# ParthaEth/GIF

Hardware: AMD Instinct MI355X
Metric: G+D train-step images/sec at 256x256, batch 32/GPU (higher is better)
Workload: dtype f32

## Files before the change

gif_amd/_lib.py:

```python
import ctypes
import os

import torch

_HERE = os.path.dirname(os.path.abspath(__file__))
LIB_PATH = os.path.join(_HERE, "libgif_hip.so")

c_int, c_i64, c_float, c_void_p = ctypes.c_int, ctypes.c_int64, ctypes.c_float, ctypes.c_void_p


def knob(name, default):
    if os.environ.get("GIF_EXPERIMENTAL", "0") in ("", "0"):
        return default
    return os.environ.get(name, default)
P = c_void_p


class ConvGeom(ctypes.Structure):
    _fields_ = [(n, ctypes.c_int32) for n in ("B", "Hb", "Wb", "Cb", "Hs", "Ws", "Cs", "KH", "KW", "stride", "pad")]


class ConvEpilogue(ctypes.Structure):
    _fields_ = [("in_scale", P), ("out_scale", P), ("bias", P), ("residual", P),
                ("act", ctypes.c_int32), ("slope", c_float), ("gain", c_float),
                ("mask_src", P), ("mask_slope", c_float), ("mask_gain", c_float),
                ("dot_src", P), ("dot", P), ("colsum", P), ("red_ws", P), ("out_f32", ctypes.c_int32)]


class LinearBankSeg(ctypes.Structure):
    _fields_ = [("w", P), ("bias", P), ("s", P), ("gs", P), ("gw", P), ("gbias", P), ("n", ctypes.c_int32), ("reserved", ctypes.c_int32)]


GP, EP = ctypes.POINTER(ConvGeom), ctypes.POINTER(ConvEpilogue)

PROTOTYPES = {
    "gif_last_error": (ctypes.c_char_p, []),
    "gif_abi_version": (c_int, []),
    "gif_f16_overflow_clear": (c_int, [P]),
    "gif_f16_overflow_or_into": (c_int, [P, P]),
    "gif_f16_overflow_watch": (c_int, [c_int]),
    "gif_set_fp32_mfma_mode": (c_int, [c_int]),
    "gif_get_fp32_mfma_mode": (c_int, []),
    "gif_rasterize_workspace_bytes": (c_i64, [c_int, c_int, c_int, c_int]),
    "gif_rasterize_assume_clean_workspace": (c_int, [P, c_int]),
    "gif_rasterize_f32": (c_int, [P, P, P, P, c_int, c_int, c_int, c_int, P, P]),
    "gif_rasterize_colors_f32": (c_int, [P, P, P, P, P, c_int, c_int, c_int, c_int, P, P]),
    "gif_rasterize_f64": (c_int, [P, P, P, P, c_int, c_int, c_int, c_int, P, P]),
    "gif_rasterize_colors_f64": (c_int, [P, P, P, P, P, c_int, c_int, c_int, c_int, P, P]),
    "gif_rasterize_colors_bwd_workspace_bytes": (c_i64, [c_int, c_int, c_int, c_int]),
    "gif_rasterize_colors_bwd_f32": (c_int, [P, P, P, P, P, P, c_int, c_int, c_int, c_int, P, P]),
    "gif_vertex_normals_f32": (c_int, [P, P, P, P, P, c_int, c_int, c_int, P]),
    "gif_vertex_normals_bwd_f32": (c_int, [P, P, P, P, P, P, P, c_int, c_int, c_int, P]),
    "gif_face_gather_bwd_f32": (c_int, [P, P, P, P, c_int, c_int, c_int, P]),
    "gif_antialias_f32": (c_int, [P] * 6 + [c_int] * 5 + [P]),
    "gif_antialias_bwd_workspace_bytes": (c_i64, [c_int, c_int, c_int, c_int]),
    "gif_antialias_bwd_f32": (c_int, [P] * 8 + [c_int] * 5 + [P, P]),
    "gif_antialias_walk_f32": (c_int, [P] * 6 + [c_int] * 6 + [P]),
    "gif_antialias_walk_bwd_f32": (c_int, [P] * 8 + [c_int] * 6 + [P, P]),
    "gif_flame_skin_f32": (c_int, [P] * 7 + [c_int] * 4 + [P]),
# ... 174 lines not shown
```

gif_amd/csrc/conv_igemm.hip:

```cpp
#include <stdlib.h>

#include <atomic>
#include <type_traits>

#include "conv_common.h"
#include "conv_route.h"

namespace {

using gif::f32x16, gif::f32x4, gif::xcd_remap;
using gif::buf_rsrc_t, gif::make_buf_rsrc, gif::buf_load_lds16;

struct GatherParams {
    const void* x;
    const void* wp;
    void* y;
    const float* in_scale;
    const float* out_scale;
    const float* bias;
    const void* residual;
    int B, Hi, Wi, Ci;
    int Ho, Wo, Co;
    int Hp, Wp;
    int os, ooy, oox;
    int is;
    int ntaps, nky, nkx, dy0, ddy, dx0, ddx, ky0, kx0, kstep, KW;
    int RP, CP;
    int act;
    float slope, gain;
    int M;
    int tiles_m, tiles_n;
    int stab_nb, stab_stride;
    const void* zero;
    int m_begin;
    int x3;
    const int* wexp;
    unsigned* gate;
    unsigned gate_gen;
    unsigned* h2_stats;
    const void* mask_src;
    const void* dot_src;
    float mask_slope, mask_gain;
    float* part_cs;
    float* part_dot;
    int part_row0;
    int part_cap;
    int no_split;
    unsigned* sat_flag;
    int out_f32;
    int pair;
    int dense;
    int t2_tx, t2_ty;
};

template <int BM, int BN, int LD, int MT, int NT, typename T = float, int THREADS = 256, bool T2D = false, int LDS_FLOATS = 0, int PFMAX = 4>
__device__ __forceinline__ void conv_epilogue(const GatherParams& p, f32x16 (&acc)[MT][NT], float* smem, int m0, int n0,
                                              int wm0, int wn0, int tid, int li, int lh, int HWp, int t2_b = 0, int t2_oy0 = 0,
                                              int t2_ox0 = 0) {
    const T* const res = static_cast<const T*>(p.residual);
    T* const yout = static_cast<T*>(p.y);
    constexpr int LDC = BN + 4;
    constexpr int ROWTAB = 3;
    constexpr int STAGE_FLOATS = LDS_FLOATS ? LDS_FLOATS : 2 * (BM + BN) * LD;
    constexpr int EPI_CHUNKS = (BM * (LDC + ROWTAB) <= STAGE_FLOATS) ? 1 : (BM / 2 * (LDC + ROWTAB) <= STAGE_FLOATS) ? 2
                               : (BM / 4 * (LDC + ROWTAB) <= STAGE_FLOATS) ? 4 : 8;
    constexpr int CR = BM / EPI_CHUNKS;
    static_assert(CR % 32 == 0 && CR * (LDC + ROWTAB) <= STAGE_FLOATS && CR <= THREADS, "epilogue chunk must fit the staging LDS");
    float* Cs = smem;
    unsigned long long* const roff = reinterpret_cast<unsigned long long*>(Cs + CR * LDC);
    int* const rsmp = reinterpret_cast<int*>(roff + CR);
    constexpr unsigned long long NO_ROW = ~0ull;
    constexpr int C4_ROW = BN / 4;
    constexpr int EROWS = THREADS / C4_ROW;
    constexpr int E_IT = CR / EROWS;
    static_assert(CR % EROWS == 0, "epilogue row mapping");
    const int e_row0 = tid / C4_ROW, e_c = (tid % C4_ROW) * 4;
    const int n = n0 + e_c;
    float4 bias4 = make_float4(0.f, 0.f, 0.f, 0.f);
    if (p.bias && n < p.Co) bias4 = *reinterpret_cast<const float4*>(p.bias + n);
    const T* const msk = static_cast<const T*>(p.mask_src);
    const T* const dsrc = static_cast<const T*>(p.dot_src);
    const bool fused = msk || dsrc || p.part_cs || p.part_dot;
    float4 cs = make_float4(0.f, 0.f, 0.f, 0.f), ds = make_float4(0.f, 0.f, 0.f, 0.f);
    int osb = 0;
    f32x4 osc0 = {1.f, 1.f, 1.f, 1.f}, osc1 = osc0;
    constexpr bool OSC = sizeof(T) == 4;
    if (OSC && p.out_scale && n < p.Co) {
        osb = T2D ? t2_b : (m0 < p.M ? m0 : p.M - 1) / HWp;
        osc0 = *reinterpret_cast<const f32x4*>(p.out_scale + (size_t)osb * p.Co + n);
        osc1 = *reinterpret_cast<const f32x4*>(p.out_scale + (size_t)(osb + 1 < p.B ? osb + 1 : osb) * p.Co + n);
    }
#pragma unroll
    for (int c = 0; c < EPI_CHUNKS; ++c) {
        __syncthreads();
        if (tid < CR) {
            int b, oy, ox;
            bool okr;
            if constexpr (T2D) {
                const int r2 = c * CR + tid;
                b = t2_b; oy = t2_oy0 + (r2 >> 4); ox = t2_ox0 + (r2 & 15);
                okr = oy < p.Hp && ox < p.Wp;
            } else {
                const int m = m0 + c * CR + tid;
                okr = m < p.M;
                const int mm = okr ? m : 0;
                b = mm / HWp;
                const int rr = mm - b * HWp;
                oy = rr / p.Wp; ox = rr - oy * p.Wp;
            }
            roff[tid] = okr ? (unsigned long long)((((size_t)b * p.Ho + (oy * p.os + p.ooy)) * p.Wo + (ox * p.os + p.oox)) * p.Co) : NO_ROW;
            rsmp[tid] = b;
        }
#pragma unroll
        for (int i = 0; i < MT; ++i) {
// ... 38 lines not shown
                            }
                        }
                    }
#pragma unroll
                    for (int k = 0; k < PF; ++k) {
                        if (!ok[k]) continue;
                        float4 v = vv[k];
                        if constexpr (sizeof(T) != 4) v = *reinterpret_cast<const float4*>(Cs + (e_row0 + (it0 + k) * EROWS) * LDC + e_c);
                        if (FUSED && dsrc) {
                            ds.x += v.x * xa[k].x; ds.y += v.y * xa[k].y; ds.z += v.z * xa[k].z; ds.w += v.w * xa[k].w;
                        }
                        if (p.out_scale) {
                            f32x4 d = bs[k] == osb ? os0 : os1;
                            if (!OSC || __builtin_expect(bs[k] > osb + 1, 0)) d = *reinterpret_cast<const f32x4*>(p.out_scale + (size_t)bs[k] * p.Co + n);
                            const float dx = d[0], dy = d[1], dz = d[2], dw = d[3];
                            v.x *= dx; v.y *= dy; v.z *= dz; v.w *= dw;
                        }
                        if (res) {
                            float4 rv = gif::load4(res + off[k]);
                            v.x += rv.x; v.y += rv.y; v.z += rv.z; v.w += rv.w;
                        }
                        v.x += bias4.x; v.y += bias4.y; v.z += bias4.z; v.w += bias4.w;
                        if (p.act) {
                            v.x = (v.x > 0.f ? v.x : v.x * p.slope) * p.gain; v.y = (v.y > 0.f ? v.y : v.y * p.slope) * p.gain;
                            v.z = (v.z > 0.f ? v.z : v.z * p.slope) * p.gain; v.w = (v.w > 0.f ? v.w : v.w * p.slope) * p.gain;
                        }
                        if (FUSED) {
                            if (msk) {
                                const float4 xs = two_src ? xb[k] : xa[k];
                                v.x *= p.mask_gain * (xs.x > 0.f ? 1.f : p.mask_slope); v.y *= p.mask_gain * (xs.y > 0.f ? 1.f : p.mask_slope);
                                v.z *= p.mask_gain * (xs.z > 0.f ? 1.f : p.mask_slope); v.w *= p.mask_gain * (xs.w > 0.f ? 1.f : p.mask_slope);
                            }
                            cs.x += v.x; cs.y += v.y; cs.z += v.z; cs.w += v.w;
                        }
                        {
                            if (sizeof(T) == 2 && p.out_f32) gif::store4(static_cast<float*>(p.y) + off[k], v);
                            else gif::store4_flag(yout + off[k], v, p.sat_flag);
                        }
                    }
                }
            };
            if (fused) rows(std::true_type{});
            else rows(std::false_type{});
        }
    }
    if (p.part_cs || p.part_dot) {
        __syncthreads();
        float4* red = reinterpret_cast<float4*>(smem);
        red[tid] = cs;
        red[THREADS + tid] = ds;
        __syncthreads();
        if (tid < C4_ROW && n < p.Co) {
            float4 a = red[tid], b = red[THREADS + tid];
#pragma unroll 4
            for (int k = 1; k < EROWS; ++k) {
                const float4 a2 = red[k * C4_ROW + tid], b2 = red[THREADS + k * C4_ROW + tid];
                a.x += a2.x; a.y += a2.y; a.z += a2.z; a.w += a2.w;
                b.x += b2.x; b.y += b2.y; b.z += b2.z; b.w += b2.w;
            }
            const int prow_i = p.part_row0 + (m0 - p.m_begin) / BM;
            const size_t prow = (size_t)prow_i * p.Co + n;
            if (prow_i < p.part_cap) {
                if (p.part_cs) *reinterpret_cast<float4*>(p.part_cs + prow) = a;
                if (p.part_dot) *reinterpret_cast<float4*>(p.part_dot + prow) = b;
            }
        }
// ... 1245 lines not shown
    if (wp_fallback) {
        const gif::H2Gate gt = gif::h2_next_gate(s);
        if (gt.err) return gt.err;
        p.gate = gt.word; p.gate_gen = gt.gen;
        p.h2_stats = gif::h2_stats_words();
    }
    return 0;
}
inline void h2_to_fallback(GatherParams& p, const void* wp3) {
    p.x3 = 1;
    p.wp = wp3;
    p.wexp = nullptr;
}

template <typename T>
int check_channels(const gif_conv_geom* g, const char* who) {
    if (sizeof(T) == 2)
        GIF_REQUIRE(g->Cb % 8 == 0 && g->Cs % 8 == 0, "%s: f16 channel counts must be multiples of 8 (Cb=%d Cs=%d)", who, g->Cb, g->Cs);
    return 0;
}

template <typename T>
route::ConvShape conv_shape(const gif_conv_geom* g, const gif_conv_epilogue* e, int x3, bool dense) {
    return route::ConvShape{g->B, g->Hb, g->Wb, g->Cb, g->Hs, g->Ws, g->Cs, g->KH, g->KW, g->stride, g->pad,
                            sizeof(T) == 2, x3, dense, e && e->in_scale, e && e->dot};
}

template <typename T>
int base_params(GatherParams& p, const void* x, const void* wp, void* y, const gif_conv_epilogue* e, int x3, int RP, const void* wp_fallback,
                hipStream_t s) {
    p.x = x; p.wp = wp; p.y = y; p.x3 = x3;
    gif::fill_epilogue(p, e);
    p.in_scale = e ? e->in_scale : nullptr;
    p.sat_flag = nullptr;
    p.out_f32 = e ? e->out_f32 : 0;
    if (sizeof(T) == 2) p.sat_flag = gif::f16_sat_flag();
    return x3 == 2 ? h2_operands(p, RP, wp, wp_fallback, s) : 0;
}

template <typename T>
int conv_run(const GatherParams& base, const route::ConvPhases& phs, const void* wp_fallback, const gif::FusedSums& sums, double flops, int d0, int d3,
             int B, long hw, hipStream_t s, const char* who, const char* twin_note) {
    const bool halo_on = halo_switch().load(std::memory_order_relaxed) != 0;
    const route::ConvRoute r = route::conv_route(phs.ph, phs.nph, sizeof(T) == 2, conv_knobs(), halo_on);
    const bool guarded = base.x3 == 2 && base.gate && wp_fallback;
    route::ConvPhases twin = phs;
    route::ConvRoute r2{};
    if (guarded) {
        for (route::ConvPhase& q : twin.ph) q.x3 = 1;
        r2 = route::conv_route(twin.ph, twin.nph, false, conv_knobs(), halo_on);
        if (!r.error && !r2.error && sums.active() && (r2.part_rows != r.part_rows || r2.tile_rows != r.tile_rows)) {
            gif::set_error("%s: the guarded bf16x3 twin tiles the op differently from the f16x2 launch (%d x %d vs %d x %d rows)%s", who,
                           r2.part_rows, r2.tile_rows, r.part_rows, r.tile_rows, twin_note);
            return GIF_ENOSUP;
        }
    }
    const route::ConvPhase& q0 = phs.ph[0];
    gif::ProfScope prof(r.family, flops, s, d0, q0.Co, q0.Ci, d3);
    GatherParams ph[4];
    for (int i = 0; i < phs.nph; ++i) {
        ph[i] = base;
        fill_phase(ph[i], phs.ph[i]);
    }
    if (r.error) return route_error(r);
    for (int i = 0; i < r.nlaunch; ++i)
        if (int rc = conv_dispatch(r.launch[i], ph, s, who)) return rc;
// ... 157 lines not shown
```

gif_amd/csrc/conv_winograd.hip:

```cpp
#include <stdlib.h>
#include <string.h>

#include "conv_common.h"
#include "wino_route.h"

namespace route = gif_wino;

namespace {

using gif::f32x16, gif::f32x4, gif::xcd_remap;

using route::WBM, route::WBN, route::WBK, route::WNSTAGE;
using route::WPAD;

__global__ void __launch_bounds__(256) wino_input_transform(const float* __restrict__ x, const float* __restrict__ scale,
                                                            float* __restrict__ V, int B, int H, int W, int C, int CP,
                                                            long ntiles_pad) {
    const int C4 = CP >> 2, TH = H >> 1, TW = W >> 1;
    const long ntiles = (long)B * TH * TW;
    const long total = ntiles * C4;
    const size_t plane = (size_t)ntiles_pad * CP;
    for (unsigned idx = blockIdx.x * blockDim.x + threadIdx.x; idx < (unsigned)total; idx += gridDim.x * blockDim.x) {
        const unsigned tile = idx / (unsigned)C4;
        const int c4 = (int)(idx - tile * (unsigned)C4);
// ... 1086 lines not shown
    return true;
}
template <int BM, int BN>
bool x3_try(const route::WinoLaunch& l, hipStream_t s, const WinoParams& p) {
    if (l.kernel != route::GEMM_X3 || l.BM != BM || l.BN != BN) return false;
    static gif::LdsAttr attr;
    gif::launch_lds(wino_gemm_x3<BM, BN>, attr, dim3(l.grid), dim3(l.threads), l.lds, s, p);
    return true;
}
template <int BM, int BN, int NST>
bool h2_try(const route::WinoLaunch& l, hipStream_t s, const WinoParams& p) {
    if (l.kernel != route::GEMM_H2 || l.BM != BM || l.BN != BN || l.NST != NST) return false;
    static gif::LdsAttr attr;
    gif::launch_lds(wino_gemm_h2<BM, BN, NST>, attr, dim3(l.grid), dim3(l.threads), l.lds, s, p);
    return true;
}

int wino_launch_one(const route::WinoLaunch& l, hipStream_t s, const WinoParams& p, const char* who) {
    const bool launched = mfma_try<4>(l, s, p) || mfma_try<2>(l, s, p) ||
                          h2_try<128, 128, 3>(l, s, p) || h2_try<128, 128, 5>(l, s, p) || h2_try<128, 128, 4>(l, s, p) ||
                          x3_try<256, 64>(l, s, p) || x3_try<128, 128>(l, s, p);
    GIF_REQUIRE(launched, "%s: the route names a kernel that is not built (gemm %d wn %d tile %dx%d stages %d)", who, l.kernel, l.WN, l.BM, l.BN,
                l.NST);
    return 0;
}

int conv3x3_winograd_impl(int mode, const float* x, const void* U, const void* U2, float* y, float* V, int B, int H, int W, int C, int Co,
                          const gif_conv_epilogue* e, gif_stream_t stream) {
    const bool split = mode != route::MODE_NATIVE, h2 = mode == route::MODE_F16X2;
    const char* const who = split ? "winograd_x3" : "winograd";
    const char* const entry = split ? "conv3x3_winograd_f32x3" : "conv3x3_winograd";
    GIF_REQUIRE(x && (U || U2) && y && V && B >= 0 && H > 0 && W > 0 && H % 2 == 0 && W % 2 == 0, "%s: bad dims (H, W must be even)", who);
    GIF_REQUIRE(C > 0 && Co > 0 && C % 4 == 0 && Co % 4 == 0, "%s: channels must be multiples of 4", who);
    if (B == 0) return 0;
    const route::WinoRoute r = route::wino_route(B, H, W, C, Co, mode, h2 && U, wino_knobs());
    GIF_REQUIRE(r.error == route::WINO_OK, "%s: tensor too large for 32-bit offsets", who);
    hipStream_t s = gif::as_stream(stream);
    double flops = 2.0 * B * H * W * 9.0 * C * Co;
    {
        gif::ProfScope prof_t(r.xform.family, 4.0 * ((double)B * H * W * C + 16.0 * r.ntiles_pad * r.CP), s, (int)((long)B * H * W), C, 0, 1);
        if (int rc = gif::winograd_input_transform(x, e ? e->in_scale : nullptr, V, B, H, W, C, s)) return rc;
    }
    gif::ProfScope prof(r.family, flops, s, (int)((long)B * H * W), Co, C, split ? 2091 : 1091);
    WinoParams p{};
    p.V = V; p.U = static_cast<const float*>(U); p.y = y;
    gif::fill_epilogue(p, e);
    p.B = B; p.H = H; p.W = W; p.Co = Co; p.RP = r.RP; p.CP = r.CP;
    p.ntiles = (int)r.ntiles; p.ntiles_pad = (int)r.ntiles_pad; p.TH = H / 2; p.TW = W / 2;
    p.tiles_m = r.primary.tiles_m; p.tiles_n = r.primary.tiles_n;
    gif::FusedSums sums;
    if (int rc = sums_begin(sums, p, e, B, H, W, Co, r.sum_tile, entry)) return rc;
    if (h2) {
        WinoParams q = p;
        q.uexp = static_cast<const int*>(U2);
        q.U = reinterpret_cast<const float*>(static_cast<const char*>(U2) + gif::h2_header_bytes(r.RP));
        if (r.has_twin) {
            const gif::H2Gate gt = gif::h2_next_gate(s);
            if (gt.err) return gt.err;
            q.gate = gt.word; q.gate_gen = gt.gen;
        }
        if (int rc = wino_launch_one(r.primary, s, q, entry)) return rc;
        if (!q.gate) {
            if (int rc = sums_finish(sums, p, B, H, W, Co, r.sum_tile, s)) return rc;
            return gif::check_launch("conv3x3_winograd_f32h2");
        }
        p.gate = q.gate; p.gate_gen = q.gate_gen; p.h2_stats = gif::h2_stats_words();
// ... 79 lines not shown
```

gif_amd/csrc/elementwise.hip:

```cpp
#include "common.h"

namespace {

__device__ __forceinline__ float wave_sum(float v) {
#pragma unroll
    for (int off = 32; off > 0; off >>= 1) v += __shfl_xor(v, off, 64);
    return v;
}

__device__ __forceinline__ float4 f4add(float4 a, float4 b) { return make_float4(a.x + b.x, a.y + b.y, a.z + b.z, a.w + b.w); }
__device__ __forceinline__ float4 f4fma(float s, float4 a, float4 c) {
    return make_float4(fmaf(s, a.x, c.x), fmaf(s, a.y, c.y), fmaf(s, a.z, c.z), fmaf(s, a.w, c.w));
}
__device__ __forceinline__ float lrelu(float v, float slope, float gain) { return (v > 0.f ? v : v * slope) * gain; }

template <typename T>
struct UpfirdnParams {
    const T* x;
    const float* k;
    T* y;
    const float* bias;
    const T* residual;
    int B, Hi, Wi, C, Ho, Wo, up, down, padx0, pady0, KH, KW, flip, act;
    float slope, gain;
// ... 583 lines not shown
    const int f = R / S, o0 = f / 2 - 1;
    long total = (long)B * R * R * C4;
    for (long idx = (long)blockIdx.x * blockDim.x + threadIdx.x; idx < total; idx += (long)gridDim.x * blockDim.x) {
        int c4 = (int)(idx % C4);
        long pix = idx / C4;
        int ix = (int)(pix % R);
        long t = pix / R;
        int iy = (int)(t % R), b = (int)(t / R);
        float4 r = make_float4(0.f, 0.f, 0.f, 0.f);
        if (f == 1) {
            r = reinterpret_cast<const float4*>(gy)[idx];
        } else {
            int ry = iy % f - o0, rx = ix % f - o0;
            if ((ry == 0 || ry == 1) && (rx == 0 || rx == 1)) {
                float4 g = reinterpret_cast<const float4*>(gy)[(((size_t)b * S + iy / f) * S + ix / f) * C4 + c4];
                r = make_float4(0.25f * g.x, 0.25f * g.y, 0.25f * g.z, 0.25f * g.w);
            }
        }
        reinterpret_cast<float4*>(gx)[idx] = r;
    }
}

const gif_ew::FirKnobs& fir_knobs() {
    static const gif_ew::FirKnobs once = gif_ew::parse_fir_knobs(gif::knob("GIF_FIR_BLOCK"));
    return once;
}

template <typename T>
int upfirdn2d_impl(const T* x, const float* k, T* y, int B, int Hi, int Wi, int C, int Ho, int Wo, int up, int down, int padx0,
                   int pady0, int KH, int KW, int flip, const gif_conv_epilogue* e, gif_stream_t stream) {
    GIF_REQUIRE(x && k && y, "upfirdn2d: null pointer");
    GIF_REQUIRE(B >= 0 && Hi > 0 && Wi > 0 && Ho > 0 && Wo > 0 && C > 0 && C % 4 == 0, "upfirdn2d: bad dims (C=%d)", C);
    GIF_REQUIRE(up >= 1 && down >= 1 && KH >= 1 && KW >= 1 && KH * KW <= 16, "upfirdn2d: bad up/down/kernel");
    if (B == 0) return 0;
    UpfirdnParams<T> p{};
    p.x = x; p.k = k; p.y = y;
    p.bias = e ? e->bias : nullptr;
    p.residual = e ? static_cast<const T*>(e->residual) : nullptr;
    p.act = e ? e->act : 0;
    p.slope = e ? e->slope : 0.f;
    p.gain = e ? e->gain : 1.f;
    p.B = B; p.Hi = Hi; p.Wi = Wi; p.C = C; p.Ho = Ho; p.Wo = Wo; p.up = up; p.down = down;
    p.padx0 = padx0; p.pady0 = pady0; p.KH = KH; p.KW = KW; p.flip = flip;
    p.sat_flag = sizeof(T) == 2 ? gif::f16_sat_flag() : nullptr;
    float* colsum_out = nullptr;
    if (e && (e->mask_src || e->colsum || e->dot || e->dot_src)) {
        GIF_REQUIRE(!e->dot && !e->dot_src, "upfirdn2d: the dot fusion is a convolution epilogue only");
        GIF_REQUIRE(up == 1 && down == 1 && KH == 4 && KW == 4, "upfirdn2d: mask / colsum fusions need the 4x4 blur form (up = down = 1)");
        GIF_REQUIRE(!e->colsum || (e->red_ws && (C & (C - 1)) == 0 && C <= 1024), "upfirdn2d: colsum needs red_ws and a power-of-two C <= 1024");
        p.mask_src = static_cast<const T*>(e->mask_src);
        p.mask_slope = e->mask_slope; p.mask_gain = e->mask_gain;
        colsum_out = e->colsum;
        p.part_cs = colsum_out ? e->red_ws : nullptr;
    }
    const gif_ew::FirRoute r = gif_ew::fir_route({B, C, Ho, Wo, up, down, padx0, pady0, KH, KW}, colsum_out != nullptr, fir_knobs());
    const dim3 grid(r.grid_x, r.grid_y);
    hipStream_t s = gif::as_stream(stream);
    const char* what = "upfirdn2d";
    switch (r.kernel) {
    case gif_ew::FIR_BLUR_ROWS:
        blur4x4_rows_kernel<T, 16, 4><<<grid, r.threads, 0, s>>>(p);
        what = "upfirdn2d(blur rows)";
        break;
    case gif_ew::FIR_BLUR_TILED:
        blur4x4_tiled_kernel<T, 2, 4><<<grid, r.threads, 0, s>>>(p);
        what = "upfirdn2d(blur)";
// ... 398 lines not shown
```

gif_amd/functional.py:

```python
import weakref

import torch
from torch.autograd import Function

from . import ops
from .ops import ConvSpec


class ActPort:
    __slots__ = ("alias", "slope", "gain", "want_bias", "parts", "y_ref")

    def __init__(self, slope, gain, want_bias):
        self.alias, self.slope, self.gain, self.want_bias = None, float(slope), float(gain), bool(want_bias)
        self.parts = []
        self.y_ref = None

    def cfg(self):
        return (self.slope, self.gain, self.want_bias, self.parts, self.y_ref)


def _observed(t):
    return t.retains_grad or bool(t._backward_hooks)


def _port_live(cfg):
    if cfg is None:
        return False
    y = cfg[4]() if cfg[4] is not None else None
    return y is None or not _observed(y)


def _file_part(parts, part):
    if not parts:
        torch.autograd.Variable._execution_engine.queue_callback(parts.clear)
    parts.append(part)


def _take_port(x, identity=False):
    port = getattr(x, "_gif_port", None)
    if (port is None or not ops.FUSE_GRAD or not torch.is_grad_enabled() or port.alias is None or not port.alias.requires_grad
            or (port.slope == 1.0 and port.gain == 1.0) != identity or _observed(x)):
        return None, None
    return port.alias, port.cfg()


_inputs_only = False


class inputs_only_backward:
    def __enter__(self):
        global _inputs_only
        self._prev, _inputs_only = _inputs_only, True

    def __exit__(self, *exc):
        global _inputs_only
        _inputs_only = self._prev


def _param_mask(*tensors):
    P = torch.nn.Parameter
    return tuple(isinstance(t, torch.Tensor) and (isinstance(t, P) or isinstance(getattr(t, "_base", None), P)) for t in tensors)


def _need(ctx, i):
    return ctx.needs_input_grad[i] and not (_inputs_only and ctx.pmask[i])


def _port_on(ctx):
    return ctx.in_port is not None and not torch.is_grad_enabled() and _port_live(ctx.in_port)


def _tag(y, alias, port):
    if port is not None:
        port.alias = alias
        port.y_ref = weakref.ref(y)
        y._gif_port = port
    return y


def _new_port(x_requires_grad, slope, gain, bias):
    if not ops.FUSE_GRAD or not torch.is_grad_enabled():
        return None
    want_bias = bias is not None and bias.requires_grad
    if slope == 1.0 and gain == 1.0 and not want_bias:
        return None
    return ActPort(slope, gain, want_bias)


def _deliver_residual(r_port, gpre, gb):
    want_b, parts = r_port[2:4]
    if want_b:
        _file_part(parts, gb if gb is not None else ops.colsum(gpre))
    return gpre


def _mask_into_port(cfg, gx, x):
    slope, gain, want_b, parts = cfg[:4]
    gxm, gb = BiasActBwdFn.apply(gx, x, want_b, slope, gain)
    if want_b:
        _file_part(parts, gb)
    return gxm


def _producer_gpre(gy, g_port, y, want_b, slope, gain, parts):
    gpre = gb = None
    if gy is not None:
        gpre, gb = BiasActBwdFn.apply(gy, y, want_b, slope, gain)
        if not want_b:
            gb = None
    if g_port is not None:
        gpre = g_port if gpre is None else gpre + g_port
        if want_b and parts:
            for part in parts:
                gb = part if gb is None else gb + part
    if parts is not None:
        parts.clear()
    return gpre, gb


class Conv2dFn(Function):

    @staticmethod
    def forward(ctx, x, w, spec, transposed, out_hw, wscale, residual=None):
        ctx.pmask = _param_mask(x, w)
        x = ops.nhwc(x)
        ctx.spec, ctx.transposed, ctx.wscale = spec, transposed, wscale
        ctx.save_for_backward(x, w)
        ctx.v = None
        epi = {} if residual is None else {"residual": ops.nhwc(residual)}
        if not transposed:
            y, v = ops.conv_fwd(x, w, spec, wscale, keep_v=True, **epi)
            ctx.v = v if ctx.needs_input_grad[1] else None
            return y
        return ops.conv_bwd_data(x, w, spec, tuple(out_hw), wscale, **epi)

    @staticmethod
    def backward(ctx, gy):
        x, w = ctx.saved_tensors
# ... 36 lines not shown
    def forward(ctx, x, w, bias, spec, wscale, slope, gain, passthrough=False, in_port=None, parts=None, x_port=None):
        ctx.set_materialize_grads(False)
        ctx.pmask = _param_mask(x, w, bias)
        x = ops.nhwc(x)
        y, v = ops.conv_fwd(x, w, spec, wscale, keep_v=True, bias=bias, act=True, slope=slope, gain=gain)
        ctx.v = v if ctx.needs_input_grad[1] else None
        ctx.cfg = (spec, wscale, slope, gain, bias is not None)
        ctx.in_port, ctx.parts = in_port, parts
        ctx.save_for_backward(x, w, y)
        return y, y.detach(), (x.view_as(x) if passthrough else None)

    @staticmethod
    def backward(ctx, gy, g_port=None, g_alias=None):
        x, w, y = ctx.saved_tensors
        spec, ws, slope, gain, has_bias = ctx.cfg
        want_b = has_bias and _need(ctx, 2)
        gx = gw = None
        port = _port_on(ctx)
        gpre, gb = _producer_gpre(gy, g_port, y, want_b, slope, gain, ctx.parts)
        if gpre is not None:
            if ctx.needs_input_grad[0]:
                gx = _conv_dgrad(gpre, w, spec, tuple(x.shape[2:]), ws, g_alias, ctx.in_port if port else None, x)
            if _need(ctx, 1):
                gw = WgradFn.apply(gpre, x, spec, w.shape[0], w.shape[1], ws, ctx.v)
        elif ctx.needs_input_grad[0] and g_alias is not None:
            gx = _mask_into_port(ctx.in_port, g_alias, x) if port else g_alias
        return (None if port else gx), gw, (gb if want_b else None), None, None, None, None, None, None, None, (gx if port else None)


def _conv_dgrad(gpre, w, spec, big_hw, ws, residual, in_port, x):
    if in_port is None:
        return Conv2dFn.apply(gpre, w, spec, True, big_hw, ws, residual)
    slope, gain, want_b, parts = in_port[:4]
    fuse = ops.GradFuse(mask_src=x, mask_slope=slope, mask_gain=gain, want_colsum=want_b)
    gx = ops.conv_bwd_data(gpre, w, spec, big_hw, ws, residual=None if residual is None else ops.nhwc(residual), fuse=fuse)
    if want_b:
        _file_part(parts, fuse.colsum)
    return gx


def conv2d_bias_act(x, w, bias, stride=1, pad=0, wscale=1.0, slope=0.2, gain=2 ** 0.5, passthrough=False):
    x_port, in_port = _take_port(x)
    port = _new_port(True, slope, gain, bias)
    y, alias, x_alias = ConvBiasActFn.apply(x, w, bias, ConvSpec(w.shape[2], w.shape[3], stride, pad), wscale, slope, gain,
                                            bool(passthrough), in_port, None if port is None else port.parts, x_port)
    _tag(y, alias, port)
    return (y, x_alias) if passthrough else y


def conv2d(x, w, stride=1, pad=0, wscale=1.0, residual=None):
    return Conv2dFn.apply(x, w, ConvSpec(w.shape[2], w.shape[3], stride, pad), False, None, wscale, residual)


def conv_transpose2d(x, w, stride, pad, out_hw, wscale=1.0):
    return Conv2dFn.apply(x, w, ConvSpec(w.shape[2], w.shape[3], stride, pad), True, tuple(out_hw), wscale, None)


class LinearNtFn(Function):

    @staticmethod
    def forward(ctx, a, b, scale, n_pad):
        ctx.scale = scale
        ctx.pmask = _param_mask(a, b)
        ctx.save_for_backward(a, b)
        return ops.linear_nt(a, b, None, scale, n_pad=n_pad)

    @staticmethod
    def backward(ctx, g):
        a, b = ctx.saved_tensors
        N, K = b.shape
        ga = LinearNnFn.apply(g, b, ctx.scale, a.shape[1]) if _need(ctx, 0) else None
# ... 400 lines not shown
def minibatch_stddev(x, group, Cy):
    if x.dtype != torch.float32:
        return MbstdFn.apply(x.float(), group, Cy).to(x.dtype)
    return MbstdFn.apply(x, group, Cy)


def _modconv_composite(x, w, s, d, spec, transposed, out_hw, wscale, residual=None, bias=None, act=None):
    z = Conv2dFn.apply(x * s.to(x.dtype)[:, :, None, None], w, spec, transposed, out_hw, wscale, None)
    if d is not None:
        z = z * d.to(z.dtype)[:, :, None, None]
    if act is None:
        return z
    slope, gain = act
    return BiasActFn.apply(z, bias, residual, slope, gain)


def _recorded_backward(inputs, needs, gy, build):
    with torch.enable_grad():
        proxies = [None if t is None else t.view_as(t) for t in inputs]
        y = build(*proxies)
        idx = [i for i, (t, n) in enumerate(zip(inputs, needs)) if n and t is not None and t.requires_grad]
        grads = torch.autograd.grad(y, [proxies[i] for i in idx], gy, create_graph=True, allow_unused=True)
    out = [None] * len(inputs)
    for i, g in zip(idx, grads):
        out[i] = g
    return out


def _modconv_dgrad_fused(g, w, spec, tr, x, s, d, ws, in_port, want_gs):
    slope, gain, want_b, parts = in_port[:4] if in_port is not None else (1.0, 1.0, False, None)
    fuse = None
    if in_port is not None or want_gs:
        fuse = ops.GradFuse(mask_src=x if in_port is not None else None, mask_slope=slope, mask_gain=gain, want_colsum=want_b,
                            dot_src=x if want_gs else None)
    if not tr:
        gx = ops.conv_bwd_data(g, w, spec, tuple(x.shape[2:]), ws, in_scale=d, out_scale=s, fuse=fuse)
    else:
        gx = ops.conv_fwd(g, w, spec, ws, in_scale=d, out_scale=s, fuse=fuse)
    if want_b:
        _file_part(parts, fuse.colsum)
    return gx, (None if fuse is None else fuse.dot)


class ModConvFn(Function):

    @staticmethod
    def forward(ctx, x, w, s, d, spec, transposed, out_hw, wscale, in_port=None, x_port=None, out_f32=False):
        x_in, s_in, d_in = x, s, d
        ctx.pmask = _param_mask(x, w, s, d)
        x = ops.nhwc(x)
        s = s.contiguous()
        d = None if d is None else d.contiguous()
        ctx.v = None
        if not transposed:
            y, v = ops.conv_fwd(x, w, spec, wscale, keep_v=True, in_scale=s, out_scale=d, out_f32=out_f32)
            ctx.v = v if ctx.needs_input_grad[1] else None
        else:
            y = ops.conv_bwd_data(x, w, spec, tuple(out_hw), wscale, in_scale=s, out_scale=d)
        ctx.spec, ctx.transposed, ctx.wscale = spec, transposed, wscale
        ctx.out_hw = tuple(y.shape[2:])
        ctx.in_port = in_port
        none = x.new_empty(())
        ctx.save_for_backward(x_in, w, s_in, d_in if d is not None else none, y if d is not None else none)
        ctx.has_d = d is not None
        return y

    @staticmethod
    def backward(ctx, gy):
        x, w, s, d, y = ctx.saved_tensors
        d = d if ctx.has_d else None
        spec, tr, ws = ctx.spec, ctx.transposed, ctx.wscale
        if torch.is_grad_enabled():
            gx, gw, gs, gd = _recorded_backward(
# ... 114 lines not shown
```

gif_amd/ops.py:

```python
import ctypes
import functools
import os
import weakref
from typing import NamedTuple, Optional

import torch

from . import _lib

CL = torch.channels_last


def _stream():
    return torch.cuda.current_stream().cuda_stream


def _device_guard(fn):
    @functools.wraps(fn)
    def wrapped(*args, **kw):
        dev = None
        for a in args + tuple(kw.values()):
            if isinstance(a, torch.Tensor) and a.is_cuda:
                if dev is None:
                    dev = a.device
# ... 40 lines not shown


def _same_dtype(a, b, what):
    if a.dtype != b.dtype:
        raise _lib.GifHipError(f"{what}: operands of different dtypes ({a.dtype} and {b.dtype})")


def empty_nhwc(B, C, H, W, device, dtype=torch.float32):
    return torch.empty((B, C, H, W), device=device, dtype=dtype, memory_format=CL)


class ConvSpec(NamedTuple):
    KH: int
    KW: int
    stride: int
    pad: int

    def small_hw(self, Hb, Wb):
        return ((Hb + 2 * self.pad - self.KH) // self.stride + 1, (Wb + 2 * self.pad - self.KW) // self.stride + 1)

    def big_hw(self, Hs, Ws):
        return ((Hs - 1) * self.stride + self.KH - 2 * self.pad, (Ws - 1) * self.stride + self.KW - 2 * self.pad)


def _geom(B, Hb, Wb, Cb, Hs, Ws, Cs, spec: ConvSpec):
    return _lib.ConvGeom(B, Hb, Wb, Cb, Hs, Ws, Cs, spec.KH, spec.KW, spec.stride, spec.pad)


FUSE_GRAD = _lib.knob("GIF_FUSE_GRAD", "1") != "0"


class GradFuse:

    def __init__(self, mask_src=None, mask_slope=1.0, mask_gain=1.0, want_colsum=False, dot_src=None):
        self.mask_src, self.mask_slope, self.mask_gain = mask_src, float(mask_slope), float(mask_gain)
        self.want_colsum, self.dot_src = bool(want_colsum), dot_src
        self.colsum = self.dot = self._ws = None


def dot_fusable(H, W, dtype=torch.float32):
    return FUSE_GRAD and dtype in (torch.float32, torch.float16) and (H * W) % 1024 == 0


def _epilogue(in_scale=None, out_scale=None, bias=None, residual=None, act=False, slope=0.2, gain=2 ** 0.5, fuse=None,
              out_bchw=None, dtype=torch.float32, out_f32=False):
    e = _lib.ConvEpilogue(_p(in_scale), _p(out_scale), _p(bias), _p(residual), 1 if act else 0, slope, gain)
    e.out_f32 = 1 if out_f32 else 0
    if fuse is not None:
        B, C, H, W = out_bchw
        for t, what in ((fuse.mask_src, "mask_src"), (fuse.dot_src, "dot_src")):
            if t is not None and (tuple(t.shape) != (B, C, H, W) or t.dtype != dtype or not t.is_contiguous(memory_format=CL)):
                raise _lib.GifHipError(f"GradFuse.{what}: expected an NHWC {dtype} tensor of shape {(B, C, H, W)}, got {tuple(t.shape)} {t.dtype}")
        e.mask_src, e.mask_slope, e.mask_gain = _p(fuse.mask_src), fuse.mask_slope, fuse.mask_gain
        e.dot_src = _p(fuse.dot_src)
        if fuse.mask_src is None and fuse.dot_src is None:
            raise _lib.GifHipError("GradFuse: nothing to fuse (the plain column sum of a gradient is ops.colsum)")
        device = fuse.mask_src.device if fuse.mask_src is not None else fuse.dot_src.device
        if fuse.dot_src is not None:
            fuse.dot = torch.empty((B, C), device=device, dtype=torch.float32)
            e.dot = fuse.dot.data_ptr()
        if fuse.want_colsum:
            fuse.colsum = torch.empty((C,), device=device, dtype=torch.float32)
            e.colsum = fuse.colsum.data_ptr()
        if fuse.dot is not None or fuse.colsum is not None:
            fuse._ws = torch.empty((_lib.load().gif_conv_epilogue_ws_floats(B * H * W, C),), device=device, dtype=torch.float32)
            e.red_ws = fuse._ws.data_ptr()
    return e


WEIGHT_CACHE = _lib.knob("GIF_WEIGHT_CACHE", "1") != "0"
_weight_cache = {}
_WEIGHT_CACHE_MAX = 512


def clear_weight_cache():
    _weight_cache.clear()


def _cached_weight_op(w, tag, build):
    if not WEIGHT_CACHE:
        return build()
    base = w._base if w._base is not None else w
    key = (id(base), tag, w.storage_offset(), tuple(w.shape), tuple(w.stride()))
    state = (base.data_ptr(), base._version)
    hit = _weight_cache.get(key)
    if hit is not None and hit[0]() is base and hit[1] == state:
        return hit[2]
# ... 169 lines not shown

def conv3x3_winograd(x, w, rows_are_out: bool, cout_act: int, wscale=1.0, keep_v=False, **epi):
    global _winograd_calls
    _winograd_calls += 1
    lib = _lib.load()
    x = nhwc(x)
    B, C, H, W = x.shape
    R, Cc, sr, sc, sky, skx = _weight_view(w, rows_are_out, cout_act, C)
    mode = winograd_mode("fwd", cout_act)

    def build():
        RP, CP = _dims(lib.gif_winograd_pack_dims if mode == "native" else lib.gif_winograd_pack_dims_x3, cout_act, C, "winograd_pack_dims")
        U = [torch.empty((lib.gif_winograd_weight_f32h2_bytes(RP, CP),), device=x.device, dtype=torch.uint8)] if mode == "f16x2" else []
        U.append(torch.empty((16, RP, CP), device=x.device, dtype=torch.float32) if mode == "native" else
                 torch.empty((16, 3, RP, CP), device=x.device, dtype=torch.bfloat16))
        _call("winograd_weight", mode, w.data_ptr(), *[u.data_ptr() for u in U], R, Cc, RP, CP, sr, sc, sky, skx, 0 if rows_are_out else 1,
              float(wscale), _stream())
        return tuple(U) if mode == "f16x2" else U[0]

    U = _cached_weight_op(w, ("wino", rows_are_out, cout_act, C, float(wscale), mode), build)
    V = torch.empty((lib.gif_winograd_workspace_floats(B, H, W, C),), device=x.device, dtype=torch.float32)
    out = empty_nhwc(B, cout_act, H, W, x.device)
    e = _epilogue(out_bchw=(B, cout_act, H, W), **epi)
    _call("conv3x3_winograd", mode, x.data_ptr(), *_weight_ptrs(U), out.data_ptr(), V.data_ptr(), B, H, W, C, cout_act, ctypes.byref(e), _stream())
    return (out, V) if keep_v else out


def _epi_check(x, epi):
    r = epi.get("residual")
    if r is not None:
        _same_dtype(x, r, "conv epilogue residual")


def _conv_direct(plan: ConvPlan, op: str, src, w, out_bchw, g, wscale, epi):
    fwd, dt = op == "conv2d_fwd", src.dtype
    if plan.mode == "f16x2":
        wp = pack_weight_h2x3(w, fwd, out_bchw[1], src.shape[1], wscale, tapdense=plan.dense)
    else:
        wp = pack_weight(w, fwd, out_bchw[1], src.shape[1], wscale, dt, x3=plan.mode == "bf16x3", tapdense=plan.dense)
    out = empty_nhwc(*out_bchw, src.device, torch.float32 if epi.get("out_f32") else dt)
    e = _epilogue(out_bchw=out_bchw, dtype=dt, **epi)
    _call(op, plan.mode, src.data_ptr(), *_weight_ptrs(wp), out.data_ptr(), ctypes.byref(g), ctypes.byref(e), _stream(), dense=plan.dense)
    return out


def conv_fwd(big, w, spec: ConvSpec, wscale=1.0, keep_v=False, **epi):
    big = nhwc(big)
    dt = big.dtype
    B, Cb, Hb, Wb = big.shape
    Cs = cpad(w.shape[0], dt)
    Hs, Ws = spec.small_hw(Hb, Wb)
    _epi_check(big, epi)
    if dt != torch.float16:
        epi.pop("out_f32", None)
    plan = conv_plan("fwd", dt, B, spec, (Hb, Wb), (Hs, Ws), Cb, Cs, epi, big.numel() * big.element_size())
    if plan.route == "winograd":
        return conv3x3_winograd(big, w, True, Cs, wscale, keep_v=keep_v, **epi)
    out = _conv_direct(plan, "conv2d_fwd", big, w, (B, Cs, Hs, Ws), _geom(B, Hb, Wb, Cb, Hs, Ws, Cs, spec), wscale, epi)
    return (out, None) if keep_v else out


def conv_bwd_data(small, w, spec: ConvSpec, big_hw, wscale=1.0, **epi):
    small = nhwc(small)
    dt = small.dtype
    B, Cs, Hs, Ws = small.shape
    Cb = cpad(w.shape[1], dt)
    Hb, Wb = big_hw
    _epi_check(small, epi)
    plan = conv_plan("dgrad", dt, B, spec, (Hb, Wb), (Hs, Ws), Cs, Cb, epi, small.numel() * small.element_size())
    if plan.route == "winograd":
        return conv3x3_winograd(small, w, False, Cb, wscale, **epi)
    return _conv_direct(plan, "conv2d_bwd_data", small, w, (B, Cb, Hb, Wb), _geom(B, Hb, Wb, Cb, Hs, Ws, Cs, spec), wscale, epi)


def pad32(c: int) -> int:
    return (c + 31) // 32 * 32


def conv3x3_winograd_wgrad(small, big, O, I, wscale=1.0, small_scale=None, big_scale=None, big_v=None):
    global _winograd_calls
    _winograd_calls += 1
    lib = _lib.load()
    small, big = nhwc(small), nhwc(big)
    B, Cs, H, W = small.shape
    Cb = big.shape[1]
    assert big.shape == (B, Cb, H, W) and O <= Cs and I <= Cb
    RP, CP = _dims(lib.gif_conv2d_wgrad_dims, pad32(Cs), pad32(Cb), "wgrad_dims")
    nsplit = lib.gif_conv3x3_winograd_wgrad_splits(B, H, W, Cs, Cb)
    dev = small.device
    nv = lib.gif_winograd_workspace_floats(B, H, W, Cb)
    if big_v is not None and big_v.numel() != nv:
        raise _lib.GifHipError(f"conv3x3_winograd_wgrad: cached V has {big_v.numel()} floats, expected {nv}")
    V = big_v if big_v is not None else torch.empty((nv,), device=dev, dtype=torch.float32)
    Mg = torch.empty((lib.gif_winograd_workspace_floats(B, H, W, Cs),), device=dev, dtype=torch.float32)
    ws = torch.empty((nsplit, 16, RP, CP), device=dev, dtype=torch.float32)
    _call("conv3x3_winograd_wgrad", winograd_mode("wgrad", Cs), None if big_v is not None else big.data_ptr(), small.data_ptr(), V.data_ptr(),
          Mg.data_ptr(), ws.data_ptr(), _p(small_scale), _p(big_scale), B, H, W, Cs, Cb, nsplit, _stream())
    dw = torch.empty((O, I, 3, 3), device=dev, dtype=torch.float32)
    so, si, sky, skx = dw.stride()
    _lib.check(lib.gif_winograd_unpack_wgrad_f32(ws.data_ptr(), dw.data_ptr(), nsplit, O, I, RP, CP, so, si, sky, skx, float(wscale),
                                                 _stream()), "winograd_unpack_wgrad")
    return dw


# ... 520 lines not shown
```

include/gif_hip.h:

```cpp
#ifndef GIF_HIP_H
#define GIF_HIP_H

#include <stdint.h>

#ifdef __cplusplus
extern "C" {
#endif

#define GIF_EINVAL (-1)
#define GIF_ENOSUP (-2)

typedef void* gif_stream_t;

const char* gif_last_error(void);
int gif_abi_version(void);

int gif_f16_overflow_clear(gif_stream_t stream);
int gif_f16_overflow_or_into(float* found_inf, gif_stream_t stream);
int gif_f16_overflow_watch(int on);

#define GIF_FP32_MFMA_NATIVE 0
#define GIF_FP32_MFMA_BF16X3 1
#define GIF_FP32_MFMA_F16X2 2
int gif_set_fp32_mfma_mode(int mode);
// ... 88 lines not shown
                            const int32_t* texel_map, const int32_t* texel_faces, const float* texel_bc, float* gimg,
                            int B, int C, int H, int W, int V, int T, gif_stream_t stream);

int gif_shade_sh_f32(const float* uv, const float* nrm, const uint8_t* mask, const float* albedo, const float* sh, float* out,
                     int B, int Ba, int H, int W, int T, float nrm_mul, float nrm_add, gif_stream_t stream);
int64_t gif_shade_sh_bwd_workspace_bytes(int B, int H, int W);
int gif_shade_sh_bwd_f32(const float* uv, const float* nrm, const uint8_t* mask, const float* albedo, const float* sh,
                         const float* g_out, float* g_uv, float* g_nrm, float* g_albedo, float* g_sh, int B, int Ba, int H,
                         int W, int T, float nrm_mul, float nrm_add, void* workspace, gif_stream_t stream);

typedef struct {
    int32_t B;
    int32_t Hb, Wb, Cb;
    int32_t Hs, Ws, Cs;
    int32_t KH, KW;
    int32_t stride;
    int32_t pad;
} gif_conv_geom;

typedef struct {
    const float* in_scale;
    const float* out_scale;
    const float* bias;
    const void* residual;
    int32_t act;
    float slope, gain;
    const void* mask_src;
    float mask_slope, mask_gain;
    const void* dot_src;
    float* dot;
    float* colsum;
    float* red_ws;
    int32_t out_f32;
} gif_conv_epilogue;
int64_t gif_conv_epilogue_ws_floats(int64_t out_rows, int cout);

int gif_conv2d_pack_dims(int cout, int cin, int* RP, int* CP);
int gif_pack_weight_f32(const float* w, float* wp, int R, int C, int KH, int KW, int RP, int CP, int64_t sr,
                        int64_t sc, int64_t sky, int64_t skx, float scale, gif_stream_t stream);
int gif_conv2d_fwd_f32(const float* big, const float* wp, float* small, const gif_conv_geom* g,
                       const gif_conv_epilogue* e, gif_stream_t stream);
int gif_conv2d_bwd_data_f32(const float* small, const float* wp, float* big, const gif_conv_geom* g,
                            const gif_conv_epilogue* e, gif_stream_t stream);
int gif_conv2d_fwd_f32x3(const float* big, const void* wp3, float* small, const gif_conv_geom* g, const gif_conv_epilogue* e,
                         gif_stream_t stream);
int gif_conv2d_bwd_data_f32x3(const float* small, const void* wp3, float* big, const gif_conv_geom* g,
                              const gif_conv_epilogue* e, gif_stream_t stream);
int gif_conv2d_fwd_f32h2(const float* big, const void* wp2, const void* wp3, float* small, const gif_conv_geom* g,
                         const gif_conv_epilogue* e, gif_stream_t stream);
int gif_conv2d_bwd_data_f32h2(const float* small, const void* wp2, const void* wp3, float* big, const gif_conv_geom* g,
                              const gif_conv_epilogue* e, gif_stream_t stream);
int gif_conv2d_fwd_f32h2_tapdense(const float* big, const void* wp2, const void* wp3, float* small, const gif_conv_geom* g,
                                  const gif_conv_epilogue* e, gif_stream_t stream);
int gif_conv2d_bwd_data_f32h2_tapdense(const float* small, const void* wp2, const void* wp3, float* big, const gif_conv_geom* g,
                                       const gif_conv_epilogue* e, gif_stream_t stream);
int gif_conv2d_fwd_f32x3_tapdense(const float* big, const void* wp3, float* small, const gif_conv_geom* g,
                                  const gif_conv_epilogue* e, gif_stream_t stream);
int gif_conv2d_bwd_data_f32x3_tapdense(const float* small, const void* wp3, float* big, const gif_conv_geom* g,
                                       const gif_conv_epilogue* e, gif_stream_t stream);
int gif_conv2d_wgrad_dims(int Cs, int Cb, int* RP, int* CP);
int gif_conv2d_wgrad_splits(const gif_conv_geom* g);
int gif_conv2d_wgrad_f32(const float* small, const float* big, float* ws, const float* small_scale,
                         const float* big_scale, const gif_conv_geom* g, int nsplit, gif_stream_t stream);
int gif_conv2d_wgrad_f32x3(const float* small, const float* big, float* ws, const float* small_scale,
                           const float* big_scale, const gif_conv_geom* g, int nsplit, gif_stream_t stream);
int gif_conv2d_wgrad_f32h2(const float* small, const float* big, float* ws, const float* small_scale,
// ... 156 lines not shown
```

Before: 178.7.

## Fuse joining of two masked input gradients into conv dgrad epilogue accumulate

When an activation feeds two consumers, the first consumer's masked input gradient is parked in a pending list and not returned to autograd. The second consumer's conv backward-data kernel then adds it in its epilogue via a new accum pointer. This removes a separate elementwise gradient-sum pass and one full read/write of the tensor. It adds bookkeeping around autograd ordering, falls back to an explicit add in the producer's backward, and is disabled on winograd and upfirdn routes.

```diff
diff --git a/gif_amd/_lib.py b/gif_amd/_lib.py
--- a/gif_amd/_lib.py
+++ b/gif_amd/_lib.py
@@ -24,7 +24,8 @@
     _fields_ = [("in_scale", P), ("out_scale", P), ("bias", P), ("residual", P),
                 ("act", ctypes.c_int32), ("slope", c_float), ("gain", c_float),
                 ("mask_src", P), ("mask_slope", c_float), ("mask_gain", c_float),
-                ("dot_src", P), ("dot", P), ("colsum", P), ("red_ws", P), ("out_f32", ctypes.c_int32)]
+                ("dot_src", P), ("dot", P), ("colsum", P), ("red_ws", P), ("out_f32", ctypes.c_int32),
+                ("accum", P)]
 
 
 class LinearBankSeg(ctypes.Structure):
diff --git a/gif_amd/csrc/conv_igemm.hip b/gif_amd/csrc/conv_igemm.hip
--- a/gif_amd/csrc/conv_igemm.hip
+++ b/gif_amd/csrc/conv_igemm.hip
@@ -43,6 +43,7 @@
     float mask_slope, mask_gain;
     float* part_cs;
     float* part_dot;
+    const void* accum;
     int part_row0;
     int part_cap;
     int no_split;
@@ -80,6 +81,7 @@
     if (p.bias && n < p.Co) bias4 = *reinterpret_cast<const float4*>(p.bias + n);
     const T* const msk = static_cast<const T*>(p.mask_src);
     const T* const dsrc = static_cast<const T*>(p.dot_src);
+    const T* const accum = static_cast<const T*>(p.accum);
     const bool fused = msk || dsrc || p.part_cs || p.part_dot;
     float4 cs = make_float4(0.f, 0.f, 0.f, 0.f), ds = make_float4(0.f, 0.f, 0.f, 0.f);
     int osb = 0;
@@ -184,6 +186,10 @@
                                 v.z *= p.mask_gain * (xs.z > 0.f ? 1.f : p.mask_slope); v.w *= p.mask_gain * (xs.w > 0.f ? 1.f : p.mask_slope);
                             }
                             cs.x += v.x; cs.y += v.y; cs.z += v.z; cs.w += v.w;
+                            if (accum) {
+                                const float4 av = gif::load4(accum + off[k]);
+                                v.x += av.x; v.y += av.y; v.z += av.z; v.w += av.w;
+                            }
                         }
                         {
                             if (sizeof(T) == 2 && p.out_f32) gif::store4(static_cast<float*>(p.y) + off[k], v);
@@ -1495,6 +1501,8 @@
     p.x = x; p.wp = wp; p.y = y; p.x3 = x3;
     gif::fill_epilogue(p, e);
     p.in_scale = e ? e->in_scale : nullptr;
+    p.accum = e ? e->accum : nullptr;
+    GIF_REQUIRE(!p.accum || p.mask_src, "conv2d: accum joins two MASKED gradients: it needs mask_src");
     p.sat_flag = nullptr;
     p.out_f32 = e ? e->out_f32 : 0;
     if (sizeof(T) == 2) p.sat_flag = gif::f16_sat_flag();
diff --git a/gif_amd/csrc/conv_winograd.hip b/gif_amd/csrc/conv_winograd.hip
--- a/gif_amd/csrc/conv_winograd.hip
+++ b/gif_amd/csrc/conv_winograd.hip
@@ -1142,6 +1142,7 @@
     const char* const entry = split ? "conv3x3_winograd_f32x3" : "conv3x3_winograd";
     GIF_REQUIRE(x && (U || U2) && y && V && B >= 0 && H > 0 && W > 0 && H % 2 == 0 && W % 2 == 0, "%s: bad dims (H, W must be even)", who);
     GIF_REQUIRE(C > 0 && Co > 0 && C % 4 == 0 && Co % 4 == 0, "%s: channels must be multiples of 4", who);
+    GIF_REQUIRE(!(e && e->accum), "%s: the post-mask accumulate is an epilogue of the direct convolution kernels only", who);
     if (B == 0) return 0;
     const route::WinoRoute r = route::wino_route(B, H, W, C, Co, mode, h2 && U, wino_knobs());
     GIF_REQUIRE(r.error == route::WINO_OK, "%s: tensor too large for 32-bit offsets", who);
diff --git a/gif_amd/csrc/elementwise.hip b/gif_amd/csrc/elementwise.hip
--- a/gif_amd/csrc/elementwise.hip
+++ b/gif_amd/csrc/elementwise.hip
@@ -639,6 +639,7 @@
     GIF_REQUIRE(x && k && y, "upfirdn2d: null pointer");
     GIF_REQUIRE(B >= 0 && Hi > 0 && Wi > 0 && Ho > 0 && Wo > 0 && C > 0 && C % 4 == 0, "upfirdn2d: bad dims (C=%d)", C);
     GIF_REQUIRE(up >= 1 && down >= 1 && KH >= 1 && KW >= 1 && KH * KW <= 16, "upfirdn2d: bad up/down/kernel");
+    GIF_REQUIRE(!(e && e->accum), "upfirdn2d: the post-mask accumulate is an epilogue of the direct convolution kernels only");
     if (B == 0) return 0;
     UpfirdnParams<T> p{};
     p.x = x; p.k = k; p.y = y;
diff --git a/gif_amd/functional.py b/gif_amd/functional.py
--- a/gif_amd/functional.py
+++ b/gif_amd/functional.py
@@ -7,12 +7,20 @@
 from .ops import ConvSpec
 
 
+class _Parts(list):
+    __slots__ = ("pending", "takers")
+
+    def __init__(self):
+        super().__init__()
+        self.pending, self.takers = [], 0
+
+
 class ActPort:
     __slots__ = ("alias", "slope", "gain", "want_bias", "parts", "y_ref")
 
     def __init__(self, slope, gain, want_bias):
         self.alias, self.slope, self.gain, self.want_bias = None, float(slope), float(gain), bool(want_bias)
-        self.parts = []
+        self.parts = _Parts()
         self.y_ref = None
 
     def cfg(self):
@@ -41,7 +49,26 @@
     if (port is None or not ops.FUSE_GRAD or not torch.is_grad_enabled() or port.alias is None or not port.alias.requires_grad
             or (port.slope == 1.0 and port.gain == 1.0) != identity or _observed(x)):
         return None, None
+    port.parts.takers += 1
     return port.alias, port.cfg()
+
+
+def _join_accum(in_port):
+    pend = in_port[3].pending
+    return pend[0] if pend else None
+
+
+def _join_result(in_port, gx, fuse):
+    parts = in_port[3]
+    pend = parts.pending
+    if fuse.joined:
+        pend.clear()
+        return gx
+    if parts.takers < 2 or pend:
+        return gx
+    torch.autograd.Variable._execution_engine.queue_callback(pend.clear)
+    pend.append(gx)
+    return None
 
 
 _inputs_only = False
@@ -104,6 +131,10 @@
 
 def _producer_gpre(gy, g_port, y, want_b, slope, gain, parts):
     gpre = gb = None
+    pend = getattr(parts, "pending", None)
+    if pend:
+        g_port = pend[0] if g_port is None else g_port + pend[0]
+        pend.clear()
     if gy is not None:
         gpre, gb = BiasActBwdFn.apply(gy, y, want_b, slope, gain)
         if not want_b:
@@ -206,11 +237,11 @@
     if in_port is None:
         return Conv2dFn.apply(gpre, w, spec, True, big_hw, ws, residual)
     slope, gain, want_b, parts = in_port[:4]
-    fuse = ops.GradFuse(mask_src=x, mask_slope=slope, mask_gain=gain, want_colsum=want_b)
+    fuse = ops.GradFuse(mask_src=x, mask_slope=slope, mask_gain=gain, want_colsum=want_b, accum=_join_accum(in_port))
     gx = ops.conv_bwd_data(gpre, w, spec, big_hw, ws, residual=None if residual is None else ops.nhwc(residual), fuse=fuse)
     if want_b:
         _file_part(parts, fuse.colsum)
-    return gx
+    return _join_result(in_port, gx, fuse)
 
 
 def conv2d_bias_act(x, w, bias, stride=1, pad=0, wscale=1.0, slope=0.2, gain=2 ** 0.5, passthrough=False):
@@ -677,13 +708,15 @@
     fuse = None
     if in_port is not None or want_gs:
         fuse = ops.GradFuse(mask_src=x if in_port is not None else None, mask_slope=slope, mask_gain=gain, want_colsum=want_b,
-                            dot_src=x if want_gs else None)
+                            dot_src=x if want_gs else None, accum=None if in_port is None else _join_accum(in_port))
     if not tr:
         gx = ops.conv_bwd_data(g, w, spec, tuple(x.shape[2:]), ws, in_scale=d, out_scale=s, fuse=fuse)
     else:
         gx = ops.conv_fwd(g, w, spec, ws, in_scale=d, out_scale=s, fuse=fuse)
     if want_b:
         _file_part(parts, fuse.colsum)
+    if in_port is not None:
+        gx = _join_result(in_port, gx, fuse)
     return gx, (None if fuse is None else fuse.dot)
 
 
diff --git a/gif_amd/ops.py b/gif_amd/ops.py
--- a/gif_amd/ops.py
+++ b/gif_amd/ops.py
@@ -96,10 +96,12 @@
 
 class GradFuse:
 
-    def __init__(self, mask_src=None, mask_slope=1.0, mask_gain=1.0, want_colsum=False, dot_src=None):
+    def __init__(self, mask_src=None, mask_slope=1.0, mask_gain=1.0, want_colsum=False, dot_src=None, accum=None):
         self.mask_src, self.mask_slope, self.mask_gain = mask_src, float(mask_slope), float(mask_gain)
         self.want_colsum, self.dot_src = bool(want_colsum), dot_src
+        self.accum = accum if mask_src is not None else None
         self.colsum = self.dot = self._ws = None
+        self.joined = False
 
 
 def dot_fusable(H, W, dtype=torch.float32):
@@ -112,11 +114,12 @@
     e.out_f32 = 1 if out_f32 else 0
     if fuse is not None:
         B, C, H, W = out_bchw
-        for t, what in ((fuse.mask_src, "mask_src"), (fuse.dot_src, "dot_src")):
+        for t, what in ((fuse.mask_src, "mask_src"), (fuse.dot_src, "dot_src"), (fuse.accum, "accum")):
             if t is not None and (tuple(t.shape) != (B, C, H, W) or t.dtype != dtype or not t.is_contiguous(memory_format=CL)):
                 raise _lib.GifHipError(f"GradFuse.{what}: expected an NHWC {dtype} tensor of shape {(B, C, H, W)}, got {tuple(t.shape)} {t.dtype}")
         e.mask_src, e.mask_slope, e.mask_gain = _p(fuse.mask_src), fuse.mask_slope, fuse.mask_gain
         e.dot_src = _p(fuse.dot_src)
+        e.accum, fuse.joined = _p(fuse.accum), fuse.accum is not None
         if fuse.mask_src is None and fuse.dot_src is None:
             raise _lib.GifHipError("GradFuse: nothing to fuse (the plain column sum of a gradient is ops.colsum)")
         device = fuse.mask_src.device if fuse.mask_src is not None else fuse.dot_src.device
@@ -352,6 +355,13 @@
         _same_dtype(x, r, "conv epilogue residual")
 
 
+def _winograd_epi(epi):
+    fuse = epi.get("fuse")
+    if fuse is not None:
+        fuse.accum = None
+    return epi
+
+
 def _conv_direct(plan: ConvPlan, op: str, src, w, out_bchw, g, wscale, epi):
     fwd, dt = op == "conv2d_fwd", src.dtype
     if plan.mode == "f16x2":
@@ -375,7 +385,7 @@
         epi.pop("out_f32", None)
     plan = conv_plan("fwd", dt, B, spec, (Hb, Wb), (Hs, Ws), Cb, Cs, epi, big.numel() * big.element_size())
     if plan.route == "winograd":
-        return conv3x3_winograd(big, w, True, Cs, wscale, keep_v=keep_v, **epi)
+        return conv3x3_winograd(big, w, True, Cs, wscale, keep_v=keep_v, **_winograd_epi(epi))
     out = _conv_direct(plan, "conv2d_fwd", big, w, (B, Cs, Hs, Ws), _geom(B, Hb, Wb, Cb, Hs, Ws, Cs, spec), wscale, epi)
     return (out, None) if keep_v else out
 
@@ -389,7 +399,7 @@
     _epi_check(small, epi)
     plan = conv_plan("dgrad", dt, B, spec, (Hb, Wb), (Hs, Ws), Cs, Cb, epi, small.numel() * small.element_size())
     if plan.route == "winograd":
-        return conv3x3_winograd(small, w, False, Cb, wscale, **epi)
+        return conv3x3_winograd(small, w, False, Cb, wscale, **_winograd_epi(epi))
     return _conv_direct(plan, "conv2d_bwd_data", small, w, (B, Cb, Hb, Wb), _geom(B, Hb, Wb, Cb, Hs, Ws, Cs, spec), wscale, epi)
 
 
diff --git a/include/gif_hip.h b/include/gif_hip.h
--- a/include/gif_hip.h
+++ b/include/gif_hip.h
@@ -144,6 +144,7 @@
     float* colsum;
     float* red_ws;
     int32_t out_f32;
+    const void* accum;
 } gif_conv_epilogue;
 int64_t gif_conv_epilogue_ws_floats(int64_t out_rows, int cout);
 
```

After: 178.7 (median of 3 runs). No clear change (+0.0%).
